# espiriki/Garbage_Classification_RCA

Hardware: AMD Instinct MI355X
Metric: train samples/sec (image+text pairs), MM-RCA ViT-B16+DistilBERT (higher is better)
Workload: dtype bf16

## Files before the change

garbage_classification_rca_amd/csrc/gemm256.hip:

```cpp
#include "common.h"
#include "lds_asm.h"
#include <type_traits>
#include <mutex>

typedef __attribute__((ext_vector_type(4))) float f32x4;
typedef __attribute__((address_space(3))) void lds_void;
typedef const __attribute__((address_space(1))) void gbl_void;

#define HT_BYTES (128 * 64 * 2)
#define STAGE_BYTES (4 * HT_BYTES)
#define LDS256_BYTES (128 * (256 * 4 + 16))
#define SLOT_A0 0
#define SLOT_A1 1
#define SLOT_B0 2
#define SLOT_B1 3

__device__ __forceinline__ int krow_f2(int row) { return (row & 3) | (((row >> 3) & 1) << 2); }

__device__ __forceinline__ void stage_half(const bf16_t* src0, const bf16_t* src1, char* lds_piece0) {
  __builtin_amdgcn_global_load_lds((gbl_void*)src0, (lds_void*)(lds_piece0), 16, 0, 0);
  __builtin_amdgcn_global_load_lds((gbl_void*)src1, (lds_void*)(lds_piece0 + 1024), 16, 0, 0);
}

template <bool F4>
// ... 618 lines not shown

#define SK_COUNTER_BYTES 4096
#define SK_MAX_UNITS 256
struct SkWorkspace { int device; void* stream; char* base; int64_t bytes; };
static SkWorkspace g_sk_ws[32];
static int g_sk_ws_n = 0;
static std::mutex g_sk_mutex;
extern "C" int64_t mmrca_gemm_streamk_workspace_bytes(void) { return SK_COUNTER_BYTES + (int64_t)SK_MAX_UNITS * 65536 * 4; }
extern "C" int mmrca_gemm_streamk_workspace(void* workspace, int64_t bytes, void* stream) {
  MMRCA_REQUIRE(workspace == nullptr || (bytes >= mmrca_gemm_streamk_workspace_bytes() && (((uintptr_t)workspace) & 15) == 0),
                "gemm_streamk_workspace: needs %lld bytes, 16-byte aligned, zero-filled", (long long)mmrca_gemm_streamk_workspace_bytes());
  int dev = 0;
  (void)hipGetDevice(&dev);
  std::lock_guard<std::mutex> lock(g_sk_mutex);
  for (int i = 0; i < g_sk_ws_n; ++i)
    if (g_sk_ws[i].stream == stream && g_sk_ws[i].device == dev) {
      if (workspace) { g_sk_ws[i].base = (char*)workspace; g_sk_ws[i].bytes = bytes; }
      else g_sk_ws[i] = g_sk_ws[--g_sk_ws_n];
      return 0;
    }
  if (!workspace || g_sk_ws_n == 32) return 0;
  g_sk_ws[g_sk_ws_n++] = SkWorkspace{dev, stream, (char*)workspace, bytes};
  return 0;
}
static char* sk_workspace_of(void* stream) {
  if (g_sk_ws_n == 0) return nullptr;
  int dev = 0;
  (void)hipGetDevice(&dev);
  std::lock_guard<std::mutex> lock(g_sk_mutex);
  for (int i = 0; i < g_sk_ws_n; ++i)
    if (g_sk_ws[i].stream == stream && g_sk_ws[i].device == dev) return g_sk_ws[i].base;
  return nullptr;
}
static int g_sk_max = 4, g_sk_min_ksteps = 24;
static bool g_sk_bf16 = false;
extern "C" int mmrca_gemm_streamk_config(int max_split, int min_ksteps, int bf16_products) {
  if (max_split >= 0) g_sk_max = max_split;
  if (min_ksteps >= 0) g_sk_min_ksteps = min_ksteps;
  if (bf16_products >= 0) g_sk_bf16 = bf16_products != 0;
  return 0;
}
int mmrca_gemm256_streamk_split(int64_t M, int64_t N, int64_t ksteps, void* stream, bool x3) {
  const int sk_max = g_sk_max;
  if ((!x3 && !g_sk_bf16) || ksteps < g_sk_min_ksteps || !sk_workspace_of(stream)) return 0;
  const int64_t tiles = ((M + 255) / 256) * (N / 256);
  const int ncu = cu_count();
  if (tiles < ncu) return 0;
  const int64_t left = tiles % ncu;
  if (left == 0) return 0;
  int64_t split = ncu / left;
  if (split > ksteps / 2) split = ksteps / 2;
  if (split > sk_max) split = sk_max;
  return split >= 2 ? (int)split : 0;
}
int64_t mmrca_gemm256_round_split(int64_t M, int64_t N) {
  const int64_t ncu = cu_count(), tm = M / 256, tn = N / 256, tiles = tm * tn;
  const int64_t rounds = tiles / ncu, rem = tiles - rounds * ncu;
  const int64_t m_split = rounds * ncu / tn;
  return rounds >= 1 && rem * 100 >= 25 * ncu && rem * 100 < 60 * ncu && m_split >= 1 && m_split < tm ? m_split * 256 : 0;
}
template <bool AK, bool BK2, int ACT, bool ADD, bool X3 = false, bool PLANES = false, bool F4 = false>
static void launch_p256(const void* A, const void* B, void* C, const void* bias, const void* addend, void* preact, int64_t M,
                        int64_t N, int64_t K, int64_t lda, int64_t ldb, int64_t ldc, float* colsum, hipStream_t st,
                        const void* A_lo = nullptr, const void* B_lo = nullptr, void* C_lo = nullptr, int nseg = 3, int pre16 = 0) {
  const int tiles_m = (int)((M + 255) / 256), tiles_n = (int)(N / 256);
  const int ncu = cu_count();
  int grid = tiles_m * tiles_n < ncu ? ((tiles_m * tiles_n) & ~7) : ncu;
  if (grid < 8) grid = 8;
  constexpr int LDS_P = 2 * STAGE_BYTES + 32768;
  int sk_split = 0;
  char* sk_ws = nullptr;
  if constexpr (!X3 || F4) {
    sk_split = mmrca_gemm256_streamk_split(M, N, K / (F4 ? 32 : 64), (void*)st, X3);
    if (sk_split >= 2) sk_ws = sk_workspace_of((void*)st);
    if (!sk_ws) sk_split = 0;
  }
  MMRCA_MAX_LDS(LDS_P, gemm_p256_k<AK, BK2, ACT, ADD, X3, PLANES, F4>);
  hipLaunchKernelGGL((gemm_p256_k<AK, BK2, ACT, ADD, X3, PLANES, F4>), dim3(grid), dim3(512), LDS_P, st, (const bf16_t*)A, (const bf16_t*)B,
                     (bf16_t*)C, (const bf16_t*)bias, (const bf16_t*)addend, (bf16_t*)preact, M, N, K, lda, ldb, ldc, tiles_m,
                     tiles_n, colsum, 0, g_mmrca_dbg, (const bf16_t*)A_lo,
                     (const bf16_t*)B_lo, (bf16_t*)C_lo, nseg, pre16, (float*)(sk_ws ? sk_ws + SK_COUNTER_BYTES : nullptr),
                     (unsigned*)sk_ws, sk_split);
}

int g_mmrca_dbg = 0;
extern "C" int mmrca_debug_set(int v) { g_mmrca_dbg = v; return 0; }

bool mmrca_gemm256_ok(int64_t M, int64_t N, int64_t K, int a_layout, int act, bool has_addend, bool has_preact, bool has_colsum, bool has_bias) {
  if (!(N % 256 == 0 && K % 64 == 0 && K >= 128 && a_layout == MMRCA_ROWK)) return false;
  if (act == MMRCA_ACT_NONE) return !has_preact && !has_colsum;
  if (act == MMRCA_ACT_GELU_SAVE_GRAD) return has_preact && !has_addend && !has_colsum;
  if (act == MMRCA_ACT_GELU) return !has_preact && !has_addend && !has_colsum;
  if (act == MMRCA_ACT_MUL) return has_preact && !has_addend && !has_bias;
  return false;
}

int mmrca_gemm256(const void* A, const void* B, void* C, const void* bias, const void* addend, void* preact, int64_t M,
                  int64_t N, int64_t K, int64_t lda, int64_t ldb, int64_t ldc, int a_layout, int b_layout, int act,
                  float* colsum, hipStream_t st) {
  const bool bk = b_layout == MMRCA_KROW;
  MMRCA_REQUIRE(mmrca_gemm256_ok(M, N, K, a_layout, act, addend != nullptr, preact != nullptr, colsum != nullptr, bias != nullptr),
                "gemm(mfma256): shape / epilogue combination not built");
  MMRCA_REQUIRE(M * lda * 2 < (1ll << 32) && (bk ? K * ldb : N * ldb) * 2 < (1ll << 32) && M * ldc * 2 < (1ll << 32),
                "gemm(mfma256): operands must be smaller than 4 GiB");
  with_bools([&](auto bk_) {
    const auto launch = [&](auto mode, auto add) {
      launch_p256<false, bk_, mode, add>(A, B, C, bias, addend, preact, M, N, K, lda, ldb, ldc, colsum, st);
    };
    using std::integral_constant;
    if (act == MMRCA_ACT_GELU_SAVE_GRAD) launch(integral_constant<int, MMRCA_ACT_GELU_SAVE_GRAD>{}, std::false_type{});
    else if (act == MMRCA_ACT_GELU) launch(integral_constant<int, MMRCA_ACT_GELU>{}, std::false_type{});
    else if (act == MMRCA_ACT_MUL) launch(integral_constant<int, MMRCA_ACT_MUL>{}, std::false_type{});
    else if (addend) launch(integral_constant<int, MMRCA_ACT_NONE>{}, std::true_type{});
    else launch(integral_constant<int, MMRCA_ACT_NONE>{}, std::false_type{});
  }, bk);
  MMRCA_CHECK_LAUNCH("gemm(mfma256)");
  return 0;
}


bool mmrca_gemm256_x3_ok(int64_t M, int64_t N, int64_t K, int a_layout, int act, bool has_addend, bool has_colsum) {
  if (!(N % 256 == 0 && K % 64 == 0 && K >= 128 && a_layout == MMRCA_ROWK) || has_addend || has_colsum) return false;
  return act == MMRCA_ACT_NONE || act == MMRCA_ACT_GELU_SAVE_GRAD;
}

int mmrca_gemm256_x3_streamk_split(int64_t M, int64_t N, int64_t K, int b_layout, bool has_a_lo, bool has_b_lo, void* stream) {
  if (!(b_layout != MMRCA_KROW && has_a_lo && has_b_lo && K % 32 == 0 && K >= 64)) return 0;
  return mmrca_gemm256_streamk_split(M, N, K / 32, stream, true);
}

int mmrca_gemm256_x3(const void* A_hi, const void* A_lo, const void* B_hi, const void* B_lo, void* C, void* C_lo, const void* bias,
                     void* preact, int64_t M, int64_t N, int64_t K, int64_t lda, int64_t ldb, int64_t ldc, int b_layout, int act,
                     hipStream_t st, int pre16) {
  const bool bk = b_layout == MMRCA_KROW;
  MMRCA_REQUIRE(M * lda * 2 < (1ll << 32) && (bk ? K * ldb : N * ldb) * 2 < (1ll << 32) && M * ldc * 4 < (1ll << 32),
                "gemm_x3(mfma256): operands must be smaller than 4 GiB");
  const bool gelu = act == MMRCA_ACT_GELU_SAVE_GRAD, planes = C_lo != nullptr;
  if (!bk && A_lo && B_lo && K % 32 == 0 && K >= 64) {
    with_bools([&](auto gelu_, auto planes_) {
      launch_p256<false, false, gelu_ ? MMRCA_ACT_GELU_SAVE_GRAD : MMRCA_ACT_NONE, false, true, planes_, true>(
          A_hi, B_hi, C, bias, nullptr, preact, M, N, K, lda, ldb, ldc, nullptr, st, A_lo, B_lo, C_lo, 3, pre16);
    }, gelu, planes);
    MMRCA_CHECK_LAUNCH("gemm_x3(mfma256,fused)");
    return 0;
  }
  with_bools([&](auto bk_, auto gelu_, auto planes_) {
    launch_p256<false, bk_, gelu_ ? MMRCA_ACT_GELU_SAVE_GRAD : MMRCA_ACT_NONE, false, true, planes_>(
        A_hi, B_hi, C, bias, nullptr, preact, M, N, K, lda, ldb, ldc, nullptr, st, A_lo, B_lo, C_lo, A_lo ? (B_lo ? 3 : 2) : 1, pre16);
  }, bk, gelu, planes);
  MMRCA_CHECK_LAUNCH("gemm_x3(mfma256)");
  return 0;
}

__global__ void __launch_bounds__(256)
splitk_reduce256_k(const float* __restrict__ slab, float* __restrict__ C, int64_t ldc, int ntiles, int tiles_n, int splits, int64_t M, int64_t N) {
  const int tile = blockIdx.x >> 6;
  const int idx = ((blockIdx.x & 63) << 8) + threadIdx.x;
  const float* src = slab + (int64_t)tile * 65536 + (int64_t)idx * 4;
  f32x4 s = *reinterpret_cast<const f32x4*>(src);
  for (int k = 1; k < splits; ++k) {
    const f32x4 v = *reinterpret_cast<const f32x4*>(src + (int64_t)k * ntiles * 65536);
    s += v;
  }
  const int w = idx >> 11, f = (idx >> 6) & 31, lane = idx & 63;
  const int a = f >> 4, b = (f >> 3) & 1, i = (f >> 1) & 3, j = f & 1;
  const int wr = w >> 2, wc = w & 3, l16 = lane & 15, g = lane >> 4;
  const int row = 128 * a + 64 * wr + 16 * i + l16, col = 128 * b + 32 * wc + 16 * j + 4 * g;
  const int tm = tile / tiles_n, tn = tile % tiles_n;
  if ((int64_t)tm * 256 + row >= M || (int64_t)tn * 256 + col >= N) return;
  float* dst = C + ((int64_t)tm * 256 + row) * ldc + (int64_t)tn * 256 + col;
  f32x4 c = *reinterpret_cast<f32x4*>(dst);
  c += s;
  *reinterpret_cast<f32x4*>(dst) = c;
}

extern "C" int64_t mmrca_gemm_splitk_workspace_bytes(int64_t M, int64_t N) {
  if (M <= 0 || N <= 0 || M % 8 || N % 8) return 0;
  const int64_t tiles = ((M + 255) / 256) * ((N + 255) / 256);
  if (tiles > 256) return 0;
  return (256 / tiles) * tiles * 65536 * 4;
}

static int gemm_splitk_impl(const void* A, const void* A_lo, const void* B, const void* B_lo, float* C, void* workspace,
                           int64_t workspace_bytes, int64_t M, int64_t N, int64_t K, int64_t lda, int64_t ldb, int64_t ldc,
                           int a_layout, int b_layout, void* stream) {
  const bool x3 = A_lo != nullptr;
  const int nseg = x3 ? (B_lo ? 3 : 2) : 1;
  MMRCA_REQUIRE(A && B && C && workspace, "gemm_splitk: null operand");
  const bool ragged = M % 256 != 0 || N % 256 != 0;
  MMRCA_REQUIRE(M > 0 && N > 0 && M % 8 == 0 && N % 8 == 0 && K >= 128 && K % 64 == 0 &&
                (!ragged || (a_layout == MMRCA_KROW && b_layout == MMRCA_KROW && !A_lo)),
                "gemm_splitk: needs K %% 64 == 0, K >= 128 and M, N multiples of 256 (K-major bf16 operands: of 8) (got M=%lld N=%lld K=%lld)",
                (long long)M, (long long)N, (long long)K);
  MMRCA_REQUIRE(lda % 8 == 0 && ldb % 8 == 0 && ldc % 4 == 0 && (((uintptr_t)A | (uintptr_t)B | (uintptr_t)C | (uintptr_t)workspace) & 15) == 0,
                "gemm_splitk: operands must be 16-byte aligned");
  MMRCA_REQUIRE(lda >= (a_layout == MMRCA_ROWK ? K : M) && ldb >= (b_layout == MMRCA_ROWK ? K : N) && ldc >= N, "gemm_splitk: leading dimension too small");
  const int tiles_m = (int)((M + 255) / 256), tiles_n = (int)((N + 255) / 256), tiles = tiles_m * tiles_n;
  MMRCA_REQUIRE(tiles <= 256, "gemm_splitk: more than 256 output tiles (use mmrca_gemm)");
  const int64_t ksteps = (int64_t)nseg * (K / 64);
  int64_t splits64 = 256 / tiles;
  if (splits64 > ksteps / 2) splits64 = ksteps / 2;
  const int splits = (int)splits64;
  const int ksteps_base = (int)(ksteps / splits), ksteps_rem = (int)(ksteps % splits);
  MMRCA_REQUIRE(workspace_bytes >= (int64_t)splits * tiles * 65536 * 4, "gemm_splitk: workspace too small (%lld < %lld bytes)",
                (long long)workspace_bytes, (long long)splits * tiles * 65536 * 4);
  hipStream_t st = (hipStream_t)stream;
  const bool ak = a_layout == MMRCA_KROW, bk = b_layout == MMRCA_KROW;
#define LSLAB(AK_, BK_, X3_)                                                                                                     \
  do {                                                                                                                           \
    MMRCA_MAX_LDS(LDS256_BYTES, gemm_mfma256_k<AK_, BK_, MODE_SLAB, X3_>); \
    hipLaunchKernelGGL((gemm_mfma256_k<AK_, BK_, MODE_SLAB, X3_>), dim3((tiles * splits + 7) / 8 * 8), dim3(512), LDS256_BYTES, st, (const bf16_t*)A,      \
                       (const bf16_t*)B, (bf16_t*)nullptr, (const bf16_t*)nullptr, (const bf16_t*)nullptr, (bf16_t*)nullptr, M, N, K, \
                       lda, ldb, ldc, tiles_m, tiles_n, ksteps_base, ksteps_rem, (float*)workspace, (float*)nullptr, splits,    \
                       (const bf16_t*)A_lo, (const bf16_t*)B_lo, nseg);                                                         \
  } while (0)
  if (x3) {
    if (!ak && !bk) LSLAB(false, false, true);
    else if (!ak && bk) LSLAB(false, true, true);
    else if (ak && !bk) LSLAB(true, false, true);
    else LSLAB(true, true, true);
  } else {
    if (!ak && !bk) LSLAB(false, false, false);
    else if (!ak && bk) LSLAB(false, true, false);
    else if (ak && !bk) LSLAB(true, false, false);
    else LSLAB(true, true, false);
  }
#undef LSLAB
  MMRCA_CHECK_LAUNCH("gemm_splitk(mfma256)");
  hipLaunchKernelGGL(splitk_reduce256_k, dim3(tiles * 64), dim3(256), 0, st, (const float*)workspace, C, ldc, tiles, tiles_n, splits, M, N);
  MMRCA_CHECK_LAUNCH("gemm_splitk(reduce)");
  return 0;
}

extern "C" int mmrca_gemm_splitk(const void* A, const void* B, float* C, void* workspace, int64_t workspace_bytes, int64_t M,
                                 int64_t N, int64_t K, int64_t lda, int64_t ldb, int64_t ldc, int a_layout, int b_layout,
                                 void* stream) {
  return gemm_splitk_impl(A, nullptr, B, nullptr, C, workspace, workspace_bytes, M, N, K, lda, ldb, ldc, a_layout, b_layout, stream);
}

extern "C" int mmrca_gemm_splitk_x3(const void* A_hi, const void* A_lo, const void* B_hi, const void* B_lo, float* C, void* workspace,
                                    int64_t workspace_bytes, int64_t M, int64_t N, int64_t K, int64_t lda, int64_t ldb, int64_t ldc,
                                    int a_layout, int b_layout, void* stream) {
  MMRCA_REQUIRE(A_lo || !B_lo, "gemm_x3(splitk): a B lo plane without an A lo plane is not a supported pass set");
  return gemm_splitk_impl(A_hi, A_lo, B_hi, B_lo, C, workspace, workspace_bytes, M, N, K, lda, ldb, ldc, a_layout, b_layout, stream);
}
```

garbage_classification_rca_amd/lib.py:

```python
from __future__ import annotations

import ctypes as C
import os
import subprocess
from typing import Optional

import torch

_HERE = os.path.dirname(os.path.abspath(__file__))
LIB_PATH = os.path.join(_HERE, "libmmrca.so")

F32, BF16 = 0, 1
ACT_NONE, ACT_GELU, ACT_GELU_BWD, ACT_GELU_SAVE_GRAD, ACT_MUL, ACT_GELU_SAVE_GRAD_BF16 = 0, 1, 2, 3, 4, 5
ROWK, KROW = 0, 1
IMPL_AUTO, IMPL_REF, IMPL_MFMA, IMPL_MFMA256, IMPL_MFMA_PERSIST, IMPL_MFMA_BK32, IMPL_MFMA_1STAGE, IMPL_MFMA_TALL, IMPL_MFMA_256W, IMPL_MFMA_256X4 = 0, 1, 2, 3, 4, 5, 6, 7, 8, 9

HEAD_FIELDS = [f"{blk}_{leaf}" for blk in ("sai", "sat", "c1", "c2")
               for leaf in ("wq", "bq", "wk", "bk", "wv", "bv", "g", "b")] + ["fin_w", "fin_b"]


class HeadPtrs(C.Structure):
    _fields_ = [(n, C.c_void_p) for n in HEAD_FIELDS]


class MmrcaError(RuntimeError):
    pass


def build_library(force: bool = False) -> str:
    src_dir = os.path.join(_HERE, "csrc")
    cmd = ["make", "-C", src_dir, "-j8"]
    if force:
        subprocess.run(["make", "-C", src_dir, "clean"], check=True, capture_output=True)
    r = subprocess.run(cmd, capture_output=True, text=True)
    if r.returncode != 0 or not os.path.exists(LIB_PATH):
        raise MmrcaError("building libmmrca.so failed:\n" + r.stdout[-4000:] + r.stderr[-4000:])
    return LIB_PATH


_lib = None

_i64, _i32, _f32, _vp, _u64 = C.c_int64, C.c_int, C.c_float, C.c_void_p, C.c_uint64
_SIGS = {
    "mmrca_gemm": [_vp] * 6 + [_i64] * 6 + [_i32] * 6 + [_vp],
    "mmrca_gemm_colsum": [_vp] * 7 + [_i64] * 6 + [_i32] * 5 + [_vp],
    "mmrca_gemm_rows": [_vp] * 7 + [_i64] * 8 + [_i32] * 5 + [_vp],
    "mmrca_gemm_splitk": [_vp] * 4 + [_i64] * 7 + [_i32] * 2 + [_vp],
    "mmrca_gemm_streamk_workspace": [_vp, _i64, _vp],
    "mmrca_gemm_streamk_config": [_i32, _i32, _i32],
    "mmrca_gemm_x3": [_vp] * 10 + [_i64] * 6 + [_i32] * 5 + [_vp],
    "mmrca_gemm_splitk_x3": [_vp] * 6 + [_i64] * 7 + [_i32] * 2 + [_vp],
    "mmrca_split_f32": [_vp, _vp, _vp, _i64, _vp],
    "mmrca_sgd_step_x3": [_vp, _vp, _vp, _vp, _i64, _f32, _f32, _f32, _vp],
    "mmrca_adamw_step_x3": [_vp] * 6 + [_i64] + [_f32] * 5 + [_i32, _f32, _vp],
    "mmrca_nchw_to_rows": [_vp, _vp, _i32, _i32, _i32, _i32, _i32, _vp],
    "mmrca_im2row3x3": [_vp, _vp, _i32, _i32, _i32, _i32, _i32, _i64, _i32, _vp],
    "mmrca_col2im3x3": [_vp, _vp, _i32, _i32, _i32, _i32, _i32, _i64, _i32, _vp],
    "mmrca_im2row3x3_tap": [_vp, _vp, _i32, _i32, _i32, _i32, _i32, _i64, _i32, _vp],
    "mmrca_col2im3x3_tap": [_vp, _vp, _i32, _i32, _i32, _i32, _i32, _i64, _i32, _vp],
    "mmrca_dwconv3x3_fwd": [_vp, _vp, _vp, _i32, _i32, _i32, _i32, _i32, _i32, _vp],
    "mmrca_dwconv3x3_bwd_ws": [_vp, _vp, _vp, _vp, _vp, _i32, _i32, _i32, _i32, _i32, _i32, _vp, _i64, _vp],
    "mmrca_dwconv3x3_bwd": [_vp, _vp, _vp, _vp, _vp, _i32, _i32, _i32, _i32, _i32, _i32, _vp],
    "mmrca_conv3x3_fwd": [_vp, _vp, _vp, _vp, _vp, _vp, _i32, _i32, _i32, _i32, _i32, _i32, _vp],
    "mmrca_conv_bn_finish": [_vp, _vp, _vp, _i32, _i32, _i32, _vp, _vp, _vp, _vp, _i32, _f32, _f32, _vp],
    "mmrca_conv3x3_wgrad": [_vp, _vp, _vp, _i32, _i32, _i32, _i32, _i32, _i32, _vp],
    "mmrca_gemm_bnstats": [_vp, _vp, _vp, _i64, _i64, _i64, _i64, _i64, _i64, _i32, _vp, _vp, _vp, _vp],
    "mmrca_bn_finish_sums": [_vp, _vp, _vp, _i64, _i64, _vp, _vp, _vp, _vp, _i32, _f32, _f32, _vp],
    "mmrca_bn_act_bwd_sums": [_vp, _vp, _vp, _vp, _vp, _vp, _vp, _vp, _vp, _vp, _i64, _i32, _i32, _i32, _i32, _vp],
    "mmrca_se_dx": [_vp, _vp, _vp, _vp, _i32, _i32, _i32, _i32, _vp, _vp, _vp, _vp, _vp, _i32, _vp, _vp],
    "mmrca_bn_act_fwd_res": [_vp, _vp, _vp, _vp, _vp, _vp, _vp, _vp, _i64, _i32, _i32, _i64, _i32, _vp],
    "mmrca_bn_moments": [_vp, _vp, _vp, _vp, _i64, _i32, _i64, _i32, _vp],
    "mmrca_bn_act_fwd_fin": [_vp] * 13 + [_i64, _i32, _i32, _i64, _f32, _f32, _i32, _vp],
    "mmrca_bn_stats": [_vp, _vp, _vp, _vp, _vp, _i64, _i32, _i64, _f32, _f32, _i32, _i32, _vp],
    "mmrca_bn_stats_ws": [_vp, _vp, _vp, _vp, _vp, _i64, _i32, _i64, _f32, _f32, _i32, _i32, _vp, _i64, _i32, _vp],
    "mmrca_bn_stats_fused": [_vp, _vp, _vp, _vp, _vp, _i64, _i32, _i64, _f32, _f32, _i32, _vp, _i32, _vp],
    "mmrca_bn_act_bwd_ws": [_vp] * 10 + [_i64, _i32, _i32, _i32, _i32, _vp, _i64, _i32, _vp],
    "mmrca_bn_act_fwd": [_vp] * 6 + [_i64, _i32, _i32, _i32, _vp],
    "mmrca_bn_act_bwd": [_vp] * 10 + [_i64, _i32, _i32, _i32, _i32, _vp],
    "mmrca_rowpool_mean": [_vp, _vp, _i32, _i32, _i32, _i32, _vp],
    "mmrca_rowpool_mean_bwd": [_vp, _vp, _i32, _i32, _i32, _i32, _i32, _vp],
    "mmrca_se_scale_fwd": [_vp, _vp, _vp, _i32, _i32, _i32, _i32, _vp],
    "mmrca_se_mlp_fwd": [_vp] * 9 + [_i32] * 4 + [_vp],
    "mmrca_se_mlp_bwd": [_vp] * 16 + [_i32] * 4 + [_vp],
    "mmrca_se_scale_bwd": [_vp] * 5 + [_i32, _i32, _i32, _i32, _vp],
    "mmrca_bias_act_fwd": [_vp, _vp, _vp, _i64, _i32, _i32, _i32, _vp],
    "mmrca_bias_act_bwd": [_vp] * 5 + [_i64, _i32, _i32, _i32, _vp],
    "mmrca_residual_add": [_vp, _vp, _vp, _vp, _i32, _i64, _i32, _vp],
    "mmrca_maxpool3x3s2_fwd": [_vp, _vp, _vp, _i32, _i32, _i32, _i32, _i32, _vp],
    "mmrca_maxpool3x3s2_bwd": [_vp, _vp, _vp, _i32, _i32, _i32, _i32, _i32, _vp],
    "mmrca_channel_gather": [_vp, _vp, _vp, _i64, _i32, _i32, _i64, _i32, _i32, _vp],
    "mmrca_channel_interleave2": [_vp, _i64, _vp, _vp, _i64, _i32, _i32, _vp],
    "mmrca_channel_deinterleave2": [_vp, _vp, _i64, _vp, _i64, _i32, _i32, _vp],
    "mmrca_image_preprocess": [_vp, _vp, _vp, _i32, _i32, _i32, _vp, _vp, _vp],
    "mmrca_image_rotate_crop": [_vp, _vp, _i32, _i32, _vp],
    "mmrca_image_resize_u8": [_vp, _vp, _vp, _i32, _i32, _i32, _vp],
    "mmrca_image_augment": [_vp, _vp, _vp, _vp, _i32, _i32, _i32, _vp, _vp, _vp],
    "mmrca_colsum_accum": [_vp, _vp, _i64, _i64, _i64, _i32, _vp],
    "mmrca_gelu_bwd": [_vp, _vp, _vp, _i64, _i32, _vp],
    "mmrca_gelu_bwd_colsum": [_vp, _vp, _vp, _vp, _i64, _i64, _i64, _i32, _vp],
    "mmrca_mha_fwd": [_vp] * 4 + [_i32] * 4 + [_f32, _f32, _u64, _vp, _i32, _i32, _vp],
    "mmrca_mha_fwd_planes": [_vp] * 6 + [_i32] * 4 + [_f32, _f32, _u64, _vp, _vp],
    "mmrca_mha_fwd_planes_in": [_vp] * 7 + [_i32] * 4 + [_f32, _f32, _u64, _vp, _vp],
    "mmrca_mha_fwd_x3": [_vp] * 6 + [_i32] * 4 + [_f32, _f32, _u64, _vp, _vp],
    "mmrca_mha_bwd": [_vp] * 6 + [_i32] * 4 + [_f32, _f32, _u64, _vp, _i32, _i32, _vp],
    "mmrca_mha_bwd_colsum": [_vp] * 7 + [_i64] + [_i32] * 4 + [_f32, _f32, _u64, _vp, _i32, _i32, _vp],
    "mmrca_mha_cross_fwd": [_vp, _i64, _vp, _i64, _vp, _i64, _vp, _i64] + [_i32] * 5 + [_f32, _f32, _u64, _i32, _i32, _vp],
    "mmrca_mha_cross_fwd_x3": [_vp, _i64, _vp, _i64, _vp, _i64, _vp, _vp, _i64] + [_i32] * 5 + [_f32, _f32, _u64, _vp],
    "mmrca_mha_cls_fwd": [_vp] * 4 + [_i32] * 4 + [_f32, _f32, _u64, _vp, _i32, _vp],
    "mmrca_mha_cls_bwd": [_vp] * 6 + [_i32] * 4 + [_f32, _f32, _u64, _vp, _i32, _vp],
    "mmrca_add_layernorm_fwd": [_vp] * 8 + [_i64, _i32, _i64, _i64, _f32, _f32, _u64, _f32, _u64, _i32, _vp],
    "mmrca_add_layernorm_fwd_x3": [_vp] * 10 + [_i64, _i32, _i64, _i64, _f32, _f32, _u64, _f32, _u64, _vp],
    "mmrca_layernorm_bwd": [_vp] * 9 + [_i64, _i32, _i64, _i64, _i64, _f32, _u64, _f32, _u64, _vp, _vp, _vp, _i32, _vp],
    "mmrca_layernorm_bwd_mixed": [_vp] * 9 + [_i64, _i32, _i64, _i64, _i64, _f32, _u64, _f32, _u64, _vp, _vp, _vp, _vp],
    "mmrca_embed_fwd": [_vp] * 6 + [_i64, _i32, _i32, _vp],
    "mmrca_embed_bwd": [_vp] * 6 + [_i64, _i32, _i32, _i32, _i32, _vp],
    "mmrca_patchify_fwd": [_vp, _vp] + [_i32] * 6 + [_vp],
    "mmrca_vit_assemble_fwd": [_vp] * 4 + [_i32] * 4 + [_vp],
    "mmrca_vit_assemble_bwd": [_vp] * 4 + [_i32] * 4 + [_vp],
    "mmrca_head_fwd": [_vp, _vp, C.POINTER(HeadPtrs), _vp] + [_i32] * 6 + [_f32, _u64, _i32, _vp],
    "mmrca_head_bwd": [_vp, _vp, _vp, C.POINTER(HeadPtrs), C.POINTER(HeadPtrs), _vp, _vp] + [_i32] * 6 + [_f32, _u64, _i32, _vp, _i64, _vp],
    "mmrca_xent_fwd_bwd": [_vp, _vp, _vp, _f32, _vp, _vp, _i32, _i32, _f32, _vp],
    "mmrca_sgd_step": [_vp, _vp, _vp, _i64, _f32, _f32, _f32, _vp],
    "mmrca_adamw_step": [_vp] * 5 + [_i64] + [_f32] * 5 + [_i32, _f32, _vp],
    "mmrca_cast_f32_to_bf16": [_vp, _vp, _i64, _vp],
    "mmrca_seed_epoch_set": [_vp, _u64, _vp],
    "mmrca_sd_rowscale": [_vp, _vp, _i32, _i32, _u64, _vp],
}
EXPORTS = sorted(list(_SIGS) + ["mmrca_last_error", "mmrca_version", "mmrca_debug_set", "mmrca_bn_flat_set", "mmrca_debug_attn_stamps", "mmrca_gemm_splitk_workspace_bytes", "mmrca_gemm_streamk_workspace_bytes",
                                  "mmrca_head_bwd_workspace_bytes", "mmrca_conv3x3_stat_slots", "mmrca_gemm_bnstats_slots"])


def load(build_if_missing: bool = False):
    global _lib
    if _lib is not None:
        return _lib
    if not os.path.exists(LIB_PATH):
        if build_if_missing:
            build_library()
        else:
            raise MmrcaError(f"{LIB_PATH} not found: the HIP extension is required (run __graft_entry__.build()); "
                             "there is no CPU fallback")
    lib = C.CDLL(LIB_PATH)
    for name, args in _SIGS.items():
        fn = getattr(lib, name)
        fn.argtypes = args
        fn.restype = C.c_int
    lib.mmrca_gemm_splitk_workspace_bytes.argtypes = [_i64, _i64]
    lib.mmrca_gemm_splitk_workspace_bytes.restype = _i64
    lib.mmrca_gemm_streamk_workspace_bytes.argtypes = []
    lib.mmrca_gemm_streamk_workspace_bytes.restype = _i64
    lib.mmrca_conv3x3_stat_slots.argtypes = [_i32, _i32, _i32]
    lib.mmrca_conv3x3_stat_slots.restype = _i64
    lib.mmrca_last_error.restype = C.c_char_p
    lib.mmrca_version.restype = C.c_int
    _lib = lib
    return lib


def _check(rc: int, what: str):
    if rc != 0:
        raise MmrcaError(f"{what} failed ({rc}): {load().mmrca_last_error().decode()}")


def dtype_code(dt: torch.dtype) -> int:
    if dt == torch.float32:
        return F32
    if dt == torch.bfloat16:
        return BF16
    raise MmrcaError(f"unsupported dtype {dt}")


def ptr(t: Optional[torch.Tensor]):
    return None if t is None else t.data_ptr()


_raw_stream = getattr(torch._C, "_cuda_getCurrentRawStream", None)
_cur_device = getattr(torch._C, "_cuda_getDevice", None)


def stream_ptr() -> int:
    if _raw_stream is not None and _cur_device is not None:
        return _raw_stream(_cur_device())
    return torch.cuda.current_stream().cuda_stream


def _dev(t: torch.Tensor, name: str):
    if not t.is_cuda:
        raise MmrcaError(f"{name}: tensor must live in HBM (got device {t.device}); the product path has no CPU fallback")


GEMM_PROFILE = None
KERNEL_PROFILE = None


class _Bracket:

    def __init__(self, kind, meta):
        self.kind, self.meta, self.on = kind, meta, KERNEL_PROFILE is not None

    def __enter__(self):
        if self.on:
            self.e0, self.e1 = torch.cuda.Event(enable_timing=True), torch.cuda.Event(enable_timing=True)
# ... 605 lines not shown
```

include/mmrca.h:

```cpp
#ifndef MMRCA_H
#define MMRCA_H
#include <stdint.h>
#ifdef __cplusplus
extern "C" {
#endif

enum { MMRCA_F32 = 0, MMRCA_BF16 = 1 };
enum { MMRCA_ACT_NONE = 0, MMRCA_ACT_GELU = 1,
       MMRCA_ACT_GELU_BWD = 2,
       MMRCA_ACT_GELU_SAVE_GRAD = 3,
       MMRCA_ACT_MUL = 4,
       MMRCA_ACT_GELU_SAVE_GRAD_BF16 = 5 };
enum { MMRCA_ROWK = 0, MMRCA_KROW = 1 };
enum { MMRCA_GEMM_AUTO = 0, MMRCA_GEMM_REF = 1, MMRCA_GEMM_MFMA = 2 ,
       MMRCA_GEMM_MFMA256 = 3 ,
       MMRCA_GEMM_MFMA_PERSIST = 4 ,
       MMRCA_GEMM_MFMA_BK32 = 5 ,
       MMRCA_GEMM_MFMA_1STAGE = 6 ,
       MMRCA_GEMM_MFMA_TALL = 7 ,
       MMRCA_GEMM_MFMA_256W = 8 ,
       MMRCA_GEMM_MFMA_256X4 = 9  };

const char* mmrca_last_error(void);
int mmrca_version(void);

int mmrca_seed_epoch_set(const uint64_t* device_value, uint64_t value, void* stream);
int mmrca_sd_rowscale(const float* p, float* out, int n, int B, uint64_t seed, void* stream);
int mmrca_debug_set(int flags);
int mmrca_bn_flat_set(int mode);
int mmrca_debug_attn_stamps(void* buf);

int mmrca_gemm(const void* A, const void* B, void* C, const void* bias, const void* addend, void* preact,
               int64_t M, int64_t N, int64_t K, int64_t lda, int64_t ldb, int64_t ldc,
               int a_layout, int b_layout, int act, int out_f32_accum, int dtype, int impl, void* stream);
int mmrca_gemm_colsum(const void* A, const void* B, void* C, const void* bias, const void* addend, void* preact,
                      float* colsum, int64_t M, int64_t N, int64_t K, int64_t lda, int64_t ldb, int64_t ldc,
                      int a_layout, int b_layout, int act, int dtype, int impl, void* stream);

int64_t mmrca_gemm_bnstats_slots(int64_t M);
int mmrca_gemm_bnstats(const void* A, const void* B, void* C, int64_t M, int64_t N, int64_t K, int64_t lda, int64_t ldb, int64_t ldc,
                       int dtype, const float* shift, float* s1, float* s2, void* stream);
int mmrca_bn_finish_sums(const float* s1, const float* s2, const float* shift, int64_t nslots, int64_t rows, float* mean, float* rstd,
                         float* running_mean, float* running_var, int C, float eps, float momentum, void* stream);
int mmrca_gemm_rows(const void* A, const void* B, void* C, const void* bias, const void* addend, void* preact,
                    float* colsum, int64_t M, int64_t N, int64_t K, int64_t lda, int64_t ldb, int64_t ldc,
                    int64_t a_rows_readable, int64_t side_rows_readable, int a_layout, int b_layout, int act, int dtype,
                    int impl, void* stream);

int64_t mmrca_gemm_streamk_workspace_bytes(void);
int mmrca_gemm_streamk_workspace(void* workspace, int64_t bytes, void* stream);
int mmrca_gemm_streamk_config(int max_split, int min_ksteps, int bf16_products);

int64_t mmrca_gemm_splitk_workspace_bytes(int64_t M, int64_t N);
int mmrca_gemm_splitk(const void* A, const void* B, float* C, void* workspace, int64_t workspace_bytes, int64_t M,
                      int64_t N, int64_t K, int64_t lda, int64_t ldb, int64_t ldc, int a_layout, int b_layout, void* stream);

int mmrca_gemm_x3(const void* A_hi, const void* A_lo, const void* B_hi, const void* B_lo, void* C, void* C_lo,
                  const void* bias, const void* addend, void* preact, float* colsum, int64_t M, int64_t N, int64_t K,
                  int64_t lda, int64_t ldb, int64_t ldc, int a_layout, int b_layout, int act, int out_f32_accum,
                  int impl, void* stream);
int mmrca_gemm_splitk_x3(const void* A_hi, const void* A_lo, const void* B_hi, const void* B_lo, float* C, void* workspace,
                         int64_t workspace_bytes, int64_t M, int64_t N, int64_t K, int64_t lda, int64_t ldb, int64_t ldc,
                         int a_layout, int b_layout, void* stream);
int mmrca_split_f32(const float* src, void* hi, void* lo, int64_t n, void* stream);

int mmrca_colsum_accum(const void* dY, float* db, int64_t M, int64_t N, int64_t ld, int dtype, void* stream);

int mmrca_gelu_bwd(const void* dG, const void* H, void* dH, int64_t n, int dtype, void* stream);
int mmrca_gelu_bwd_colsum(const void* dG, const void* H, void* dH, float* db, int64_t M, int64_t N, int64_t ld,
                          int dtype, void* stream);

int mmrca_nchw_to_rows(const float* images, void* x, int B, int C, int H, int W, int dtype, void* stream);
int mmrca_im2row3x3(const void* x, void* col, int B, int H, int W, int C, int stride, int64_t ldk, int dtype, void* stream);
int mmrca_col2im3x3(const void* dcol, void* dx, int B, int H, int W, int C, int stride, int64_t ldk, int dtype, void* stream);
int mmrca_im2row3x3_tap(const void* x, void* col, int B, int H, int W, int C, int stride, int64_t ldk, int dtype, void* stream);
int mmrca_col2im3x3_tap(const void* dcol, void* dx, int B, int H, int W, int C, int stride, int64_t ldk, int dtype, void* stream);
int64_t mmrca_conv3x3_stat_slots(int B, int H, int W);
int mmrca_conv3x3_fwd(const void* x, const void* w_tap, void* z, float* part_mean, float* part_m2, float* part_cnt, int B, int H,
                      int W, int Cin, int Cout, int dtype, void* stream);
int mmrca_conv_bn_finish(float* part_mean, float* part_m2, float* part_cnt, int B, int H, int W, float* mean, float* rstd,
                         float* running_mean, float* running_var, int C, float eps, float momentum, void* stream);
int mmrca_conv3x3_wgrad(const void* dz, const void* x, float* dw_tap, int B, int H, int W, int Cin, int Cout, int dtype,
                        void* stream);
int mmrca_dwconv3x3_fwd(const void* x, const void* w, void* y, int B, int H, int W, int C, int stride, int dtype, void* stream);
int mmrca_dwconv3x3_bwd(const void* dy, const void* x, const void* w, void* dx, float* dw, int B, int H, int W, int C, int stride,
                        int dtype, void* stream);
int mmrca_dwconv3x3_bwd_ws(const void* dy, const void* x, const void* w, void* dx, float* dw, int B, int H, int W, int C, int stride,
                           int dtype, void* ws, int64_t ws_bytes, void* stream);
int mmrca_bn_stats(const void* x, float* mean, float* rstd, float* running_mean, float* running_var, int64_t rows, int C,
                   int64_t ld, float eps, float momentum, int train, int dtype, void* stream);
int mmrca_bn_stats_fused(const void* x, float* mean, float* rstd, float* running_mean, float* running_var, int64_t rows, int C,
                         int64_t ld, float eps, float momentum, int dtype, int* tickets, int flags, void* stream);
int mmrca_bn_stats_ws(const void* x, float* mean, float* rstd, float* running_mean, float* running_var, int64_t rows, int C,
                      int64_t ld, float eps, float momentum, int train, int dtype, void* ws, int64_t ws_bytes, int flags, void* stream);
int mmrca_bn_act_fwd(const void* x, const float* mean, const float* rstd, const void* gamma, const void* beta, void* y,
                     int64_t rows, int C, int act, int dtype, void* stream);
int mmrca_bn_act_fwd_res(const void* x, const float* mean, const float* rstd, const void* gamma, const void* beta, const void* res,
                         const float* rowscale, void* out, int64_t rows, int C, int act, int64_t rows_per_sample, int dtype, void* stream);
int mmrca_bn_moments(const void* x, float* s1, float* s2, float* shift, int64_t rows, int C, int64_t ld, int dtype, void* stream);
int mmrca_bn_act_fwd_fin(const void* x, const float* s1, const float* s2, const float* shift, const void* gamma, const void* beta,
                         const void* res, const float* rowscale, void* y, float* mean_out, float* rstd_out, float* running_mean,
                         float* running_var, int64_t rows, int C, int act, int64_t rows_per_sample, float eps, float momentum, int dtype,
                         void* stream);
int mmrca_bn_act_bwd(const void* dy, const void* x, const float* mean, const float* rstd, const void* gamma, const void* beta,
                     void* dx, float* dgamma, float* dbeta, float* scratch, int64_t rows, int C, int act, int train, int dtype,
                     void* stream);
int mmrca_bn_act_bwd_ws(const void* dy, const void* x, const float* mean, const float* rstd, const void* gamma, const void* beta,
                        void* dx, float* dgamma, float* dbeta, float* scratch, int64_t rows, int C, int act, int train, int dtype,
                        void* ws, int64_t ws_bytes, int flags, void* stream);
int mmrca_bn_act_bwd_sums(const void* dy, const void* x, const float* mean, const float* rstd, const void* gamma, const void* beta,
                          void* dx, float* dgamma, float* dbeta, float* sums, int64_t rows, int C, int act, int train, int dtype,
                          void* stream);
int mmrca_rowpool_mean(const void* x, void* out, int B, int HW, int C, int dtype, void* stream);
int mmrca_rowpool_mean_bwd(const void* dpool, void* dx, int B, int HW, int C, int accumulate, int dtype, void* stream);
int mmrca_se_mlp_fwd(const void* pooled, const void* w1, const void* b1, const void* w2, const void* b2, void* h_pre, void* h,
                     void* s_pre, void* s, int B, int c, int sq, int dtype, void* stream);
int mmrca_se_mlp_bwd(const void* ds, const void* pooled, const void* h_pre, const void* h, const void* s_pre, const void* w1,
                     const void* b1, const void* w2, const void* b2, void* ds_pre, void* dh_pre, void* dpool, float* gw1,
                     float* gb1, float* gw2, float* gb2, int B, int c, int sq, int dtype, void* stream);
int mmrca_se_scale_fwd(const void* x, const void* s, void* y, int B, int HW, int C, int dtype, void* stream);
int mmrca_se_scale_bwd(const void* dy, const void* x, const void* s, void* dx, void* ds, int B, int HW, int C, int dtype, void* stream);
int mmrca_se_dx(const void* dy, const void* s, const void* dpool, void* dx, int B, int HW, int C, int dtype, const void* z,
                const float* mean, const float* rstd, const void* gamma, const void* beta, int act, float* sums, void* stream);
int mmrca_bias_act_fwd(const void* x, const void* bias, void* y, int64_t rows, int C, int act, int dtype, void* stream);
int mmrca_bias_act_bwd(const void* dy, const void* x, const void* bias, void* dx, float* dbias, int64_t rows, int C, int act,
                       int dtype, void* stream);
int mmrca_residual_add(const void* a, const void* branch, const float* rowscale, void* out, int B, int64_t per_sample, int dtype,
                       void* stream);
int mmrca_maxpool3x3s2_fwd(const void* x, void* y, void* argmax, int B, int H, int W, int C, int dtype, void* stream);
int mmrca_maxpool3x3s2_bwd(const void* dy, const void* argmax, void* dx, int B, int H, int W, int C, int dtype, void* stream);
int mmrca_channel_interleave2(const void* a, int64_t lda, const void* b, void* out, int64_t rows, int bf, int dtype, void* stream);
int mmrca_channel_deinterleave2(const void* dout, void* d_even, int64_t ld_even, void* d_odd, int64_t rows, int bf, int dtype, void* stream);
int mmrca_channel_gather(const void* in, const int* map, void* out, int64_t rows, int Cin, int Cout, int64_t ld_out, int col0,
                         int dtype, void* stream);

int mmrca_mha_fwd(const void* qkv, const int32_t* key_mask, void* out, float* lse,
                  int B, int H, int S, int dh, float scale, float drop_p, uint64_t drop_seed,
                  const int32_t* cu_seqlens, int dtype, int impl, void* stream);
int mmrca_mha_bwd(const void* qkv, const int32_t* key_mask, const void* out, const void* dout, const float* lse,
                  void* dqkv, int B, int H, int S, int dh, float scale, float drop_p, uint64_t drop_seed,
                  const int32_t* cu_seqlens, int dtype, int impl, void* stream);
int mmrca_mha_fwd_planes(const void* qkv, const int32_t* key_mask, void* out, void* out_hi, void* out_lo, float* lse,
                         int B, int H, int S, int dh, float scale, float drop_p, uint64_t drop_seed,
                         const int32_t* cu_seqlens, void* stream);
int mmrca_mha_fwd_planes_in(const void* qkv_hi, const void* qkv_lo, const int32_t* key_mask, void* out, void* out_hi, void* out_lo,
                            float* lse, int B, int H, int S, int dh, float scale, float drop_p, uint64_t drop_seed,
                            const int32_t* cu_seqlens, void* stream);
int mmrca_mha_fwd_x3(const void* qkv_hi, const void* qkv_lo, const int32_t* key_mask, void* out_hi, void* out_lo, float* lse,
                     int B, int H, int S, int dh, float scale, float drop_p, uint64_t drop_seed, const int32_t* cu_seqlens, void* stream);
int mmrca_mha_cross_fwd_x3(const float* q, int64_t ldq, const float* k, int64_t ldk, const float* v, int64_t ldv, void* out_hi,
                           void* out_lo, int64_t ldo, int B, int H, int Sq, int Skv, int dh, float scale, float drop_p,
                           uint64_t drop_seed, void* stream);
int mmrca_mha_bwd_colsum(const void* qkv, const int32_t* key_mask, const void* out, const void* dout, const float* lse,
                         void* dqkv, float* dqkv_colsum, int64_t total_rows, int B, int H, int S, int dh, float scale,
                         float drop_p, uint64_t drop_seed, const int32_t* cu_seqlens, int dtype, int impl, void* stream);
int mmrca_mha_cross_fwd(const void* q, int64_t ldq, const void* k, int64_t ldk, const void* v, int64_t ldv, void* out,
                        int64_t ldo, int B, int H, int Sq, int Skv, int dh, float scale, float drop_p, uint64_t drop_seed,
                        int dtype, int impl, void* stream);
int mmrca_mha_cls_fwd(const void* qkv, const int32_t* key_mask, void* out, float* lse,
                      int B, int H, int S, int dh, float scale, float drop_p, uint64_t drop_seed,
                      const int32_t* cu_seqlens, int dtype, void* stream);
int mmrca_mha_cls_bwd(const void* qkv, const int32_t* key_mask, const void* out, const void* dout, const float* lse,
                      void* dqkv, int B, int H, int S, int dh, float scale, float drop_p, uint64_t drop_seed,
                      const int32_t* cu_seqlens, int dtype, void* stream);

int mmrca_add_layernorm_fwd(const void* x, const void* res, const void* gamma, const void* beta,
                            void* sum_out, void* y, float* mean, float* rstd,
                            int64_t rows, int D, int64_t ld_x, int64_t ld_y, float eps,
                            float in_drop_p, uint64_t in_drop_seed, float out_drop_p, uint64_t out_drop_seed,
                            int dtype, void* stream);
int mmrca_add_layernorm_fwd_x3(const void* x, const void* res, const void* gamma, const void* beta,
                               void* sum_out, void* y, void* y_hi, void* y_lo, float* mean, float* rstd,
                               int64_t rows, int D, int64_t ld_x, int64_t ld_y, float eps,
                               float in_drop_p, uint64_t in_drop_seed, float out_drop_p, uint64_t out_drop_seed, void* stream);
int mmrca_layernorm_bwd(const void* dy, const void* s, const void* gamma, const float* mean, const float* rstd,
                        const void* dres, void* ds, float* dgamma, float* dbeta,
                        int64_t rows, int D, int64_t ld_dy, int64_t ld_s, int64_t ld_ds,
                        float dy_drop_p, uint64_t dy_drop_seed, float branch_drop_p, uint64_t branch_drop_seed,
                        void* dbranch, float* dcol, float* dcol_branch, int dtype, void* stream);
int mmrca_layernorm_bwd_mixed(const void* dy, const float* s, const void* gamma, const float* mean, const float* rstd,
                              const void* dres, void* ds, float* dgamma, float* dbeta,
                              int64_t rows, int D, int64_t ld_dy, int64_t ld_s, int64_t ld_ds,
                              float dy_drop_p, uint64_t dy_drop_seed, float branch_drop_p, uint64_t branch_drop_seed,
                              void* dbranch, float* dcol, float* dcol_branch, void* stream);

int mmrca_embed_fwd(const int32_t* ids, const int32_t* pos_ids, const void* word, const void* pos,
                    const void* type_row, void* out, int64_t rows, int D, int dtype, void* stream);
int mmrca_embed_bwd(const void* dout, const int32_t* ids, const int32_t* pos_ids, float* dword, float* dpos,
                    float* dtype_row, int64_t rows, int D, int pad_id, int pos_pad_id, int dtype, void* stream);

int mmrca_patchify_fwd(const float* images, void* patches, int B, int C, int Himg, int Wimg, int P, int dtype, void* stream);
int mmrca_vit_assemble_fwd(const void* proj, const void* cls, const void* pos, void* x, int B, int nP, int D, int dtype, void* stream);
int mmrca_vit_assemble_bwd(const void* dx, void* dproj, float* dcls, float* dpos, int B, int nP, int D, int dtype, void* stream);

typedef struct {
  const float *sai_wq, *sai_bq, *sai_wk, *sai_bk, *sai_wv, *sai_bv, *sai_g, *sai_b;
  const float *sat_wq, *sat_bq, *sat_wk, *sat_bk, *sat_wv, *sat_bv, *sat_g, *sat_b;
  const float *c1_wq, *c1_bq, *c1_wk, *c1_bk, *c1_wv, *c1_bv, *c1_g, *c1_b;
  const float *c2_wq, *c2_bq, *c2_wk, *c2_bk, *c2_wv, *c2_bv, *c2_g, *c2_b;
  const float *fin_w, *fin_b;
} MmrcaHeadWeights;
typedef struct {
  float *sai_wq, *sai_bq, *sai_wk, *sai_bk, *sai_wv, *sai_bv, *sai_g, *sai_b;
  float *sat_wq, *sat_bq, *sat_wk, *sat_bk, *sat_wv, *sat_bv, *sat_g, *sat_b;
  float *c1_wq, *c1_bq, *c1_wk, *c1_bk, *c1_wv, *c1_bv, *c1_g, *c1_b;
  float *c2_wq, *c2_bq, *c2_wk, *c2_bk, *c2_wv, *c2_bv, *c2_g, *c2_b;
  float *fin_w, *fin_b;
} MmrcaHeadGrads;
// ... 63 lines not shown
```

Measured before the change: 7085.

## Add 4-wave 256x256 split-K slab kernel with 5-slot LDS pipeline

Adds a new split-K GEMM kernel that uses 4 waves per 256x256 tile, each wave owning a 128x128 sub-tile, instead of the prior 8-wave kernel. It uses a 5-slot LDS ring fed by direct global-to-LDS loads, with double-buffered register fragments interleaved with MFMA groups. The reduce kernel is templated to match the new slab layout. The new path is the default for K-major, unpadded, non-x3 operands and can be switched off through a new config entry point. The intent is more register-level reuse per wave and less barrier overhead, at the cost of heavy register and accumulator pressure and only one workgroup per CU.

Result: no change. 7108 (median of 6 runs) (+0.3%).

```diff
diff --git a/garbage_classification_rca_amd/csrc/gemm256.hip b/garbage_classification_rca_amd/csrc/gemm256.hip
--- a/garbage_classification_rca_amd/csrc/gemm256.hip
+++ b/garbage_classification_rca_amd/csrc/gemm256.hip
@@ -794,6 +794,156 @@
   return 0;
 }
 
+#define W4_SLOT_BYTES 32768
+#define W4_SLOTS 5
+#define W4_LDS_BYTES (W4_SLOTS * W4_SLOT_BYTES)
+__global__ void __launch_bounds__(256, 1)
+gemm_w4_slab_k(const bf16_t* __restrict__ A, const bf16_t* __restrict__ B, int64_t lda, int64_t ldb, int tiles_m, int tiles_n,
+               int ksteps_base, int ksteps_rem, float* __restrict__ slab, int splits) {
+  extern __shared__ __attribute__((aligned(16))) char smem[];
+  const int wave = __builtin_amdgcn_readfirstlane(threadIdx.x >> 6), lane = threadIdx.x & 63;
+  const int nwg = tiles_m * tiles_n, total = nwg * splits, per_xcd = (total + 7) >> 3;
+  const int idx = ((int)blockIdx.x & 7) * per_xcd + ((int)blockIdx.x >> 3);
+  if (((int)blockIdx.x >> 3) >= per_xcd || idx >= total) return;
+  const int yb = idx / nwg, wgid = idx - yb * nwg;
+  const int tm = wgid / tiles_n, tn = wgid - tm * tiles_n;
+  const int kt0 = yb * ksteps_base + (yb < ksteps_rem ? yb : ksteps_rem);
+  const int nh = 2 * (ksteps_base + (yb < ksteps_rem ? 1 : 0));
+
+  unsigned oa[2], ob[2];
+#pragma unroll
+  for (int ii = 0; ii < 2; ++ii) {
+    oa[ii] = (unsigned)(2 * (piece_src<true>(A, lda, (int64_t)tm * 256, (int64_t)1 << 40, 2 * wave + ii, lane) - A) + (int64_t)kt0 * 128 * lda);
+    ob[ii] = (unsigned)(2 * (piece_src<true>(B, ldb, (int64_t)tn * 256, (int64_t)1 << 40, 2 * wave + ii, lane) - B) + (int64_t)kt0 * 128 * ldb);
+  }
+  const unsigned a_step = (unsigned)(64 * lda), b_step = (unsigned)(64 * ldb);
+  const char* hbase[4] = {reinterpret_cast<const char*>(A), reinterpret_cast<const char*>(A) + 256,
+                          reinterpret_cast<const char*>(B), reinterpret_cast<const char*>(B) + 256};
+#pragma unroll
+  for (int s = 0; s < 4; ++s) asm volatile("" : "+s"(hbase[s]));
+  char* const my_piece = smem + wave * 2048;
+  int dma_slot = 0;
+#define W4_DMA(n)                                                                                                     \
+  do {                                                                                                                \
+    constexpr int s_ = (n) & 3, ii_ = (n) >> 2;                                                                       \
+    const char* src_ = hbase[s_] + (s_ < 2 ? oa[ii_] : ob[ii_]);                                                      \
+    __builtin_amdgcn_global_load_lds((gbl_void*)src_, (lds_void*)(my_piece + dma_slot + s_ * 8192 + ii_ * 1024), 16, 0, 0); \
+  } while (0)
+#define W4_DMA_NEXT()                                                                                                 \
+  do {                                                                                                                \
+    oa[0] += a_step; oa[1] += a_step; ob[0] += b_step; ob[1] += b_step;                                               \
+    dma_slot = dma_slot == (W4_SLOTS - 1) * W4_SLOT_BYTES ? 0 : dma_slot + W4_SLOT_BYTES;                             \
+  } while (0)
+
+  const unsigned lds0 = (unsigned)(uintptr_t)(lds_void*)smem;
+  unsigned abase[8], bbase[8];
+  {
+    const int g = lane >> 4, l16 = lane & 15, q = l16 >> 2, p = l16 & 3, row = 8 * g + q;
+    const unsigned a_slot = (unsigned)(wave >> 1) * 8192, b_slot = 16384 + (unsigned)(wave & 1) * 8192;
+#pragma unroll
+    for (int f = 0; f < 8; ++f) {
+      const unsigned off = row * 256 + ((f ^ krow_f2(row)) << 5) + p * 8;
+      abase[f] = lds0 + a_slot + off;
+      bbase[f] = lds0 + b_slot + off;
+    }
+  }
+  int read_slot = 0;
+#define W4_READ_NEXT()                                                                                                \
+  do {                                                                                                                \
+    const unsigned d_ = read_slot == (W4_SLOTS - 1) * W4_SLOT_BYTES ? 0u - (unsigned)((W4_SLOTS - 1) * W4_SLOT_BYTES) : (unsigned)W4_SLOT_BYTES; \
+    read_slot = read_slot == (W4_SLOTS - 1) * W4_SLOT_BYTES ? 0 : read_slot + W4_SLOT_BYTES;                          \
+    _Pragma("unroll") for (int f = 0; f < 8; ++f) { abase[f] += d_; bbase[f] += d_; }                                 \
+  } while (0)
+  Frag<true> fa[2][8], fb[2][8];
+  f32x4 acc[8][8];
+#pragma unroll
+  for (int i = 0; i < 8; ++i)
+#pragma unroll
+    for (int j = 0; j < 8; ++j) {
+      acc[i][j] = (f32x4){0.f, 0.f, 0.f, 0.f};
+      asm volatile("" : "+a"(acc[i][j]));
+    }
+
+#define W4_READ(RS, r)                                                                                                \
+  do {                                                                                                                \
+    if ((r) < 8) read_frag<true, 0>(fa[RS][(r) & 7], abase[(r) & 7]);                                                 \
+    else read_frag<true, 0>(fb[RS][(r) & 7], bbase[(r) & 7]);                                                         \
+  } while (0)
+#define W4_WAIT(RS)                                                                                                   \
+  do {                                                                                                                \
+    asm volatile("s_waitcnt lgkmcnt(0)" : "+v"(fa[RS][0].lo), "+v"(fa[RS][0].hi), "+v"(fa[RS][1].lo), "+v"(fa[RS][1].hi), \
+                 "+v"(fa[RS][2].lo), "+v"(fa[RS][2].hi), "+v"(fa[RS][3].lo), "+v"(fa[RS][3].hi), "+v"(fa[RS][4].lo),   \
+                 "+v"(fa[RS][4].hi), "+v"(fa[RS][5].lo), "+v"(fa[RS][5].hi), "+v"(fa[RS][6].lo), "+v"(fa[RS][6].hi),    \
+                 "+v"(fa[RS][7].lo), "+v"(fa[RS][7].hi) :: "memory");                                                   \
+    asm volatile("" : "+v"(fb[RS][0].lo), "+v"(fb[RS][0].hi), "+v"(fb[RS][1].lo), "+v"(fb[RS][1].hi),                  \
+                 "+v"(fb[RS][2].lo), "+v"(fb[RS][2].hi), "+v"(fb[RS][3].lo), "+v"(fb[RS][3].hi), "+v"(fb[RS][4].lo),   \
+                 "+v"(fb[RS][4].hi), "+v"(fb[RS][5].lo), "+v"(fb[RS][5].hi), "+v"(fb[RS][6].lo), "+v"(fb[RS][6].hi),    \
+                 "+v"(fb[RS][7].lo), "+v"(fb[RS][7].hi) :: "memory");                                                   \
+  } while (0)
+#define W4_GROUP(KS, q, RD, DM)                                                                                       \
+  do {                                                                                                                \
+    _Pragma("unroll") for (int u = 0; u < 4; ++u)                                                                     \
+      acc[(q) >> 1][4 * ((q) & 1) + u] = __builtin_amdgcn_mfma_f32_16x16x32_bf16(                                     \
+          frag_val(fb[KS][4 * ((q) & 1) + u]), frag_val(fa[KS][(q) >> 1]), acc[(q) >> 1][4 * ((q) & 1) + u], 0, 0, 0); \
+    if ((RD) && (q) < 8) { W4_READ((KS) ^ 1, 2 * (q)); W4_READ((KS) ^ 1, 2 * (q) + 1); }                              \
+    if ((DM) && ((q) & 1) == 0) W4_DMA((q) >> 1);                                                                     \
+    __builtin_amdgcn_sched_barrier(0);                                                                                \
+  } while (0)
+#define W4_PHASE(KS, RD, DM, VM)                                                                                      \
+  do {                                                                                                                \
+    W4_GROUP(KS, 0, RD, DM); W4_GROUP(KS, 1, RD, DM); W4_GROUP(KS, 2, RD, DM); W4_GROUP(KS, 3, RD, DM);               \
+    W4_GROUP(KS, 4, RD, DM); W4_GROUP(KS, 5, RD, DM); W4_GROUP(KS, 6, RD, DM); W4_GROUP(KS, 7, RD, DM);               \
+    W4_GROUP(KS, 8, RD, DM); W4_GROUP(KS, 9, RD, DM); W4_GROUP(KS, 10, RD, DM); W4_GROUP(KS, 11, RD, DM);             \
+    W4_GROUP(KS, 12, RD, DM); W4_GROUP(KS, 13, RD, DM); W4_GROUP(KS, 14, RD, DM); W4_GROUP(KS, 15, RD, DM);           \
+    if (DM) W4_DMA_NEXT();                                                                                            \
+    if (RD) W4_WAIT((KS) ^ 1);                                                                                        \
+    VMCNT(VM);                                                                                                        \
+    BARRIER();                                                                                                        \
+    W4_READ_NEXT();                                                                                                   \
+    __builtin_amdgcn_sched_barrier(0);                                                                                \
+  } while (0)
+
+#pragma unroll
+  for (int n = 0; n < 4; ++n) {
+    W4_DMA(0); W4_DMA(1); W4_DMA(2); W4_DMA(3); W4_DMA(4); W4_DMA(5); W4_DMA(6); W4_DMA(7);
+    W4_DMA_NEXT();
+  }
+  VMCNT(16);
+  BARRIER();
+  __builtin_amdgcn_sched_barrier(0);
+#pragma unroll
+  for (int r = 0; r < 16; ++r) W4_READ(0, r);
+  W4_WAIT(0);
+  W4_READ_NEXT();
+  __builtin_amdgcn_sched_barrier(0);
+
+  for (int h = 0; h < nh - 4; h += 2) {
+    W4_PHASE(0, 1, 1, 16);
+    W4_PHASE(1, 1, 1, 16);
+  }
+  W4_PHASE(0, 1, 0, 8);
+  W4_PHASE(1, 1, 0, 0);
+  W4_PHASE(0, 1, 0, 0);
+  W4_GROUP(1, 0, 0, 0); W4_GROUP(1, 1, 0, 0); W4_GROUP(1, 2, 0, 0); W4_GROUP(1, 3, 0, 0);
+  W4_GROUP(1, 4, 0, 0); W4_GROUP(1, 5, 0, 0); W4_GROUP(1, 6, 0, 0); W4_GROUP(1, 7, 0, 0);
+  W4_GROUP(1, 8, 0, 0); W4_GROUP(1, 9, 0, 0); W4_GROUP(1, 10, 0, 0); W4_GROUP(1, 11, 0, 0);
+  W4_GROUP(1, 12, 0, 0); W4_GROUP(1, 13, 0, 0); W4_GROUP(1, 14, 0, 0); W4_GROUP(1, 15, 0, 0);
+#undef W4_PHASE
+#undef W4_GROUP
+#undef W4_WAIT
+#undef W4_READ
+#undef W4_READ_NEXT
+#undef W4_DMA_NEXT
+#undef W4_DMA
+
+  float* dst = slab + ((int64_t)yb * nwg + wgid) * 65536 + wave * 16384 + lane * 4;
+#pragma unroll
+  for (int i = 0; i < 8; ++i)
+#pragma unroll
+    for (int j = 0; j < 8; ++j) *reinterpret_cast<f32x4*>(dst + (i * 8 + j) * 256) = acc[i][j];
+}
+
+template <bool W4>
 __global__ void __launch_bounds__(256)
 splitk_reduce256_k(const float* __restrict__ slab, float* __restrict__ C, int64_t ldc, int ntiles, int tiles_n, int splits, int64_t M, int64_t N) {
   const int tile = blockIdx.x >> 6;
@@ -804,10 +954,19 @@
     const f32x4 v = *reinterpret_cast<const f32x4*>(src + (int64_t)k * ntiles * 65536);
     s += v;
   }
-  const int w = idx >> 11, f = (idx >> 6) & 31, lane = idx & 63;
-  const int a = f >> 4, b = (f >> 3) & 1, i = (f >> 1) & 3, j = f & 1;
-  const int wr = w >> 2, wc = w & 3, l16 = lane & 15, g = lane >> 4;
-  const int row = 128 * a + 64 * wr + 16 * i + l16, col = 128 * b + 32 * wc + 16 * j + 4 * g;
+  const int lane = idx & 63, l16 = lane & 15, g = lane >> 4;
+  int row, col;
+  if constexpr (W4) {
+    const int w = idx >> 12, f = (idx >> 6) & 63;
+    row = 128 * (w >> 1) + 16 * (f >> 3) + l16;
+    col = 128 * (w & 1) + 16 * (f & 7) + 4 * g;
+  } else {
+    const int w = idx >> 11, f = (idx >> 6) & 31;
+    const int a = f >> 4, b = (f >> 3) & 1, i = (f >> 1) & 3, j = f & 1;
+    const int wr = w >> 2, wc = w & 3;
+    row = 128 * a + 64 * wr + 16 * i + l16;
+    col = 128 * b + 32 * wc + 16 * j + 4 * g;
+  }
   const int tm = tile / tiles_n, tn = tile % tiles_n;
   if ((int64_t)tm * 256 + row >= M || (int64_t)tn * 256 + col >= N) return;
   float* dst = C + ((int64_t)tm * 256 + row) * ldc + (int64_t)tn * 256 + col;
@@ -821,6 +980,18 @@
   const int64_t tiles = ((M + 255) / 256) * ((N + 255) / 256);
   if (tiles > 256) return 0;
   return (256 / tiles) * tiles * 65536 * 4;
+}
+
+static int g_splitk_kernel = MMRCA_SPLITK_AUTO;
+extern "C" int mmrca_gemm_splitk_config(int kernel) {
+  MMRCA_REQUIRE(kernel == MMRCA_SPLITK_AUTO || kernel == MMRCA_SPLITK_8WAVE || kernel == MMRCA_SPLITK_4WAVE,
+                "gemm_splitk_config: unknown kernel %d", kernel);
+  g_splitk_kernel = kernel;
+  return 0;
+}
+static bool splitk_uses_w4(int64_t M, int64_t N, int64_t K, int a_layout, int b_layout, bool x3) {
+  const bool built = !x3 && a_layout == MMRCA_KROW && b_layout == MMRCA_KROW && M % 256 == 0 && N % 256 == 0;
+  return built && g_splitk_kernel != MMRCA_SPLITK_8WAVE;
 }
 
 static int gemm_splitk_impl(const void* A, const void* A_lo, const void* B, const void* B_lo, float* C, void* workspace,
@@ -848,6 +1019,16 @@
                 (long long)workspace_bytes, (long long)splits * tiles * 65536 * 4);
   hipStream_t st = (hipStream_t)stream;
   const bool ak = a_layout == MMRCA_KROW, bk = b_layout == MMRCA_KROW;
+  if (splitk_uses_w4(M, N, K, a_layout, b_layout, x3)) {
+    MMRCA_REQUIRE(K * lda * 2 < (1ll << 32) && K * ldb * 2 < (1ll << 32), "gemm_splitk(w4): operands must be smaller than 4 GiB");
+    MMRCA_MAX_LDS(W4_LDS_BYTES, gemm_w4_slab_k);
+    hipLaunchKernelGGL(gemm_w4_slab_k, dim3((tiles * splits + 7) / 8 * 8), dim3(256), W4_LDS_BYTES, st, (const bf16_t*)A,
+                       (const bf16_t*)B, lda, ldb, tiles_m, tiles_n, ksteps_base, ksteps_rem, (float*)workspace, splits);
+    MMRCA_CHECK_LAUNCH("gemm_splitk(w4)");
+    hipLaunchKernelGGL(splitk_reduce256_k<true>, dim3(tiles * 64), dim3(256), 0, st, (const float*)workspace, C, ldc, tiles, tiles_n, splits, M, N);
+    MMRCA_CHECK_LAUNCH("gemm_splitk(reduce)");
+    return 0;
+  }
 #define LSLAB(AK_, BK_, X3_)                                                                                                     \
   do {                                                                                                                           \
     MMRCA_MAX_LDS(LDS256_BYTES, gemm_mfma256_k<AK_, BK_, MODE_SLAB, X3_>); \
@@ -869,7 +1050,7 @@
   }
 #undef LSLAB
   MMRCA_CHECK_LAUNCH("gemm_splitk(mfma256)");
-  hipLaunchKernelGGL(splitk_reduce256_k, dim3(tiles * 64), dim3(256), 0, st, (const float*)workspace, C, ldc, tiles, tiles_n, splits, M, N);
+  hipLaunchKernelGGL(splitk_reduce256_k<false>, dim3(tiles * 64), dim3(256), 0, st, (const float*)workspace, C, ldc, tiles, tiles_n, splits, M, N);
   MMRCA_CHECK_LAUNCH("gemm_splitk(reduce)");
   return 0;
 }
diff --git a/garbage_classification_rca_amd/lib.py b/garbage_classification_rca_amd/lib.py
--- a/garbage_classification_rca_amd/lib.py
+++ b/garbage_classification_rca_amd/lib.py
@@ -14,6 +14,7 @@
 ACT_NONE, ACT_GELU, ACT_GELU_BWD, ACT_GELU_SAVE_GRAD, ACT_MUL, ACT_GELU_SAVE_GRAD_BF16 = 0, 1, 2, 3, 4, 5
 ROWK, KROW = 0, 1
 IMPL_AUTO, IMPL_REF, IMPL_MFMA, IMPL_MFMA256, IMPL_MFMA_PERSIST, IMPL_MFMA_BK32, IMPL_MFMA_1STAGE, IMPL_MFMA_TALL, IMPL_MFMA_256W, IMPL_MFMA_256X4 = 0, 1, 2, 3, 4, 5, 6, 7, 8, 9
+SPLITK_AUTO, SPLITK_8WAVE, SPLITK_4WAVE = 0, 1, 2
 
 HEAD_FIELDS = [f"{blk}_{leaf}" for blk in ("sai", "sat", "c1", "c2")
                for leaf in ("wq", "bq", "wk", "bk", "wv", "bv", "g", "b")] + ["fin_w", "fin_b"]
@@ -48,6 +49,7 @@
     "mmrca_gemm_splitk": [_vp] * 4 + [_i64] * 7 + [_i32] * 2 + [_vp],
     "mmrca_gemm_streamk_workspace": [_vp, _i64, _vp],
     "mmrca_gemm_streamk_config": [_i32, _i32, _i32],
+    "mmrca_gemm_splitk_config": [_i32],
     "mmrca_gemm_x3": [_vp] * 10 + [_i64] * 6 + [_i32] * 5 + [_vp],
     "mmrca_gemm_splitk_x3": [_vp] * 6 + [_i64] * 7 + [_i32] * 2 + [_vp],
     "mmrca_split_f32": [_vp, _vp, _vp, _i64, _vp],
diff --git a/include/mmrca.h b/include/mmrca.h
--- a/include/mmrca.h
+++ b/include/mmrca.h
@@ -54,6 +54,8 @@
 int64_t mmrca_gemm_splitk_workspace_bytes(int64_t M, int64_t N);
 int mmrca_gemm_splitk(const void* A, const void* B, float* C, void* workspace, int64_t workspace_bytes, int64_t M,
                       int64_t N, int64_t K, int64_t lda, int64_t ldb, int64_t ldc, int a_layout, int b_layout, void* stream);
+enum { MMRCA_SPLITK_AUTO = 0, MMRCA_SPLITK_8WAVE = 1, MMRCA_SPLITK_4WAVE = 2 };
+int mmrca_gemm_splitk_config(int kernel);
 
 int mmrca_gemm_x3(const void* A_hi, const void* A_lo, const void* B_hi, const void* B_lo, void* C, void* C_lo,
                   const void* bias, const void* addend, void* preact, float* colsum, int64_t M, int64_t N, int64_t K,
```
